# Abhipray/audio-codec

Measured on AMD Instinct MI355X. Metric: audio channel-frames/s encode (48 kHz, 1024-line long blocks, 128 kb/s/ch), higher is better.
Workload: dtype f64

## Files before the change

### audio-codec_amd/_lib.py

```python
import ctypes
import os

HERE = os.path.dirname(os.path.abspath(__file__))
LIB_PATH = os.environ.get("PACX_LIB") or os.path.join(HERE, "libpacx.so")

PACX_ABI_VERSION = 7
PCM_I16, PCM_F64 = 0, 1
FLAG_LAST, FLAG_CUR, FLAG_NEXT = 1, 2, 4
ST_SHORT, ST_ZERO_SUBBLOCK, ST_ALLOC_CAP, ST_VQ_UNDEFINED, ST_GUARD, ST_MALFORMED = 1, 2, 4, 8, 16, 32
ST_REF_RAISES = 64
ST_RATE_CAP = 128
RATE_STEP = 32
RATE_TARGET_GRID = 64
BAND_CAND = 16
PROFILE_MAX = 8193
SEG_CF_MAX = 1 << 40
E_ARG, E_UNSUPPORTED = -1, -2
REF_SCALAR_SBR_ERROR = "'numpy.int64' object does not support item assignment"
MAX_BANDS = 32
SUB = 8

c_double_p = ctypes.POINTER(ctypes.c_double)
c_int32_p = ctypes.POINTER(ctypes.c_int32)


class PacxSmrTables(ctypes.Structure):
    _fields_ = [
        ("hann", ctypes.c_void_p),
        ("tw_cos", ctypes.c_void_p),
        ("tw_sin", ctypes.c_void_p),
        ("fft_norm", ctypes.c_double),
        ("fft_freq_step", ctypes.c_double),
        ("bark", ctypes.c_void_p),
        ("quiet", ctypes.c_void_p),
        ("band_lower", ctypes.c_void_p),
        ("band_lines", ctypes.c_void_p),
        ("n_bands", ctypes.c_int32),
    ]


class PacxConfig(ctypes.Structure):
    _fields_ = [
        ("abi_version", ctypes.c_int32),
        ("device", ctypes.c_int32),
        ("sample_rate", ctypes.c_int32),
        ("n_lines_long", ctypes.c_int32),
        ("n_lines_short", ctypes.c_int32),
        ("n_scale_bits", ctypes.c_int32),
        ("n_mant_size_bits", ctypes.c_int32),
# ... 49 lines not shown
    "pacx_abi_version": (ctypes.c_int, []),
    "pacx_create": (ctypes.c_int, [ctypes.POINTER(PacxConfig), ctypes.POINTER(_P)]),
    "pacx_destroy": (None, [_P]),
    "pacx_last_error": (ctypes.c_char_p, [_P]),
    "pacx_band_stride": (ctypes.c_int, [_P]),
    "pacx_payload_stride": (ctypes.c_int, [_P]),
    "pacx_reserve": (ctypes.c_int, [_P, ctypes.c_int64]),
    "pacx_tables_exact": (ctypes.c_int, [_P]),
    "pacx_default_bands": (ctypes.c_int, [ctypes.c_int, ctypes.c_int, c_int32_p, c_int32_p]),
    "pacx_mdct_batch": (ctypes.c_int, [_P, ctypes.POINTER(PacxPcm), _P, ctypes.c_int, _P, _P, _P]),
    "pacx_smr_batch": (ctypes.c_int, [_P, ctypes.POINTER(PacxPcm), _P, ctypes.c_int, _P, _P, _P, _P]),
    "pacx_bitalloc_batch": (ctypes.c_int, [_P, ctypes.c_int64, ctypes.c_int, _P, ctypes.c_int, _P, _P, _P, _P]),
    "pacx_quantize_batch": (ctypes.c_int, [_P, ctypes.c_int64, _P, _P, _P, ctypes.c_int, _P, _P, _P]),
    "pacx_encode_batch": (ctypes.c_int, [_P, ctypes.POINTER(PacxPcm), _P, _P, _P, _P, _P, _P, _P]),
    "pacx_encode_pack_batch": (ctypes.c_int, [_P, ctypes.POINTER(PacxPcm), _P, _P, _P, _P, _P, _P, _P, _P, _P]),
    "pacx_encode_vq_batch": (ctypes.c_int, [_P, ctypes.POINTER(PacxPcm), _P, _P, _P, _P, _P, _P, _P, _P,
                                            ctypes.c_int32, _P]),
    "pacx_pack_batch": (ctypes.c_int, [_P, ctypes.c_int64, ctypes.c_int, _P, _P, _P, _P, _P, _P, _P, _P, _P]),
    "pacx_gather_body": (ctypes.c_int, [_P, ctypes.c_int64, _P, _P, _P, ctypes.c_int64, _P, _P]),
    "pacx_window_batch": (ctypes.c_int, [_P, ctypes.c_int, ctypes.c_int64, _P, _P, _P]),
    "pacx_window_table_batch": (ctypes.c_int, [_P, _P, ctypes.c_int, ctypes.c_int64, _P, _P, _P]),
    "pacx_quantize_uniform": (ctypes.c_int, [_P, ctypes.c_int64, _P, ctypes.c_int, _P, _P]),
    "pacx_scale_factor": (ctypes.c_int, [_P, ctypes.c_int64, _P, ctypes.c_int, ctypes.c_int, _P, _P]),
    "pacx_mantissa": (ctypes.c_int, [_P, ctypes.c_int64, _P, ctypes.c_int, ctypes.c_int, ctypes.c_int, _P, _P]),
    "pacx_dequantize_uniform": (ctypes.c_int, [_P, ctypes.c_int64, _P, ctypes.c_int, _P, _P]),
    "pacx_dequantize": (ctypes.c_int, [_P, ctypes.c_int64, _P, ctypes.c_int, ctypes.c_int, ctypes.c_int, _P, _P]),
    "pacx_mantissa_fp": (ctypes.c_int, [_P, ctypes.c_int64, _P, ctypes.c_int, ctypes.c_int, ctypes.c_int, _P, _P]),
    "pacx_dequantize_fp": (ctypes.c_int, [_P, ctypes.c_int64, _P, ctypes.c_int, ctypes.c_int, ctypes.c_int, _P, _P]),
    "pacx_imdct_batch": (ctypes.c_int, [_P, ctypes.c_int64, ctypes.c_int, _P, _P, _P]),
    "pacx_mdct_direct_batch": (ctypes.c_int, [_P, ctypes.c_int64, ctypes.c_int, ctypes.c_int, ctypes.c_int, _P, _P, _P]),
    "pacx_transient_detect_f64": (ctypes.c_int, [_P, ctypes.c_int64, ctypes.c_int, ctypes.c_int, _P, ctypes.c_double, _P, _P]),
    "pacx_unpack_batch": (ctypes.c_int, [_P, ctypes.c_int64, _P, ctypes.c_int, _P, _P, _P, _P, _P, _P, _P, _P, _P]),
    "pacx_set_side_fork": (ctypes.c_int, [_P, ctypes.c_int]),
    "pacx_smr_generic_batch": (ctypes.c_int, [_P, ctypes.c_int64, ctypes.c_int, _P, _P, ctypes.POINTER(PacxSmrTables), _P, _P,
                                              _P, _P]),
    "pacx_decode_batch": (ctypes.c_int, [_P, ctypes.c_int64, ctypes.c_int, _P, _P, _P, _P, _P, _P, _P, _P]),
    "pacx_decode_sbr_batch": (ctypes.c_int, [_P, ctypes.c_int64, ctypes.c_int, _P, _P, _P, _P, _P, ctypes.c_int, _P, _P,
                                             _P, _P, _P]),
    "pacx_decode_vq_batch": (ctypes.c_int, [_P, ctypes.c_int64, ctypes.c_int, _P, ctypes.c_int, _P, _P, _P, _P, _P,
                                            _P, _P, _P, _P, _P]),
    "pacx_transient_flags": (ctypes.c_int, [_P, ctypes.POINTER(PacxPcm), _P, _P, _P]),
    "pacx_bitalloc_generic": (ctypes.c_int, [_P, ctypes.c_int64, ctypes.c_int, _P, _P, ctypes.c_int, _P, _P, _P]),
    "pacx_index_body": (ctypes.c_int, [_P, _P, ctypes.c_int64, ctypes.c_int, ctypes.c_int, ctypes.c_int64, _P, _P, _P, _P]),
    "pacx_overlap_add_pcm": (ctypes.c_int, [_P, ctypes.c_int64, ctypes.c_int, _P, _P, ctypes.c_int, _P, _P]),
    "pacx_nmr_batch": (ctypes.c_int, [_P, ctypes.POINTER(PacxPcm), _P, _P, _P, _P, _P, _P, _P, _P]),
    "pacx_nmr_summary": (ctypes.c_int, [_P, ctypes.c_int64, ctypes.c_int, _P, _P, _P, _P]),
    "pacx_encode_pack_nmr_batch": (ctypes.c_int, [_P, ctypes.POINTER(PacxPcm), _P, ctypes.c_double, ctypes.c_double,
                                                  _P, _P, _P, _P, _P, _P, _P, _P, _P]),
    "pacx_encode_pack_budget_batch": (ctypes.c_int, [_P, ctypes.POINTER(PacxPcm), _P, _P, _P, _P, _P, _P, _P, _P, _P,
                                                     _P]),
    "pacx_rate_curve_layout": (ctypes.c_int, [_P, ctypes.c_double, c_int32_p, c_int32_p]),
    "pacx_rate_curve_batch": (ctypes.c_int, [_P, ctypes.POINTER(PacxPcm), _P, ctypes.c_double, ctypes.c_int32, _P, _P, _P,
                                             _P]),
    "pacx_rate_solve": (ctypes.c_int, [_P, ctypes.c_int64, ctypes.c_int32, ctypes.c_int32, _P, _P, _P, ctypes.c_int64,
                                       ctypes.c_double, ctypes.c_double, _P, _P, _P, _P, _P]),
    "pacx_band_curve_batch": (ctypes.c_int, [_P, ctypes.POINTER(PacxPcm), _P, ctypes.c_double, _P, _P, _P, _P]),
    "pacx_band_pick": (ctypes.c_int, [_P, ctypes.c_int64, _P, _P, _P, ctypes.c_double, _P, _P, _P, _P]),
    "pacx_band_solve": (ctypes.c_int, [_P, ctypes.c_int64, _P, _P, _P, ctypes.c_int64, ctypes.c_double, ctypes.c_double,
                                       _P, _P, _P, _P, _P]),
    "pacx_band_profile": (ctypes.c_int, [_P, ctypes.c_int64, _P, _P, _P, ctypes.c_double, ctypes.c_double, _P, _P]),
    "pacx_profile_solve": (ctypes.c_int, [_P, _P, ctypes.c_int64, ctypes.c_double, ctypes.c_double, _P, _P]),
    "pacx_band_profile_segments": (ctypes.c_int, [_P, ctypes.c_int64, _P, _P, _P, ctypes.c_int64, ctypes.c_int64,
                                                  ctypes.c_double, ctypes.c_double, _P, _P]),
    "pacx_profile_solve_segments": (ctypes.c_int, [_P, ctypes.c_int64, _P, _P, ctypes.c_double, ctypes.c_double, _P, _P,
                                                   _P]),
    "pacx_profile_clamp_add": (ctypes.c_int, [_P, ctypes.c_int64, _P, _P, ctypes.c_double, ctypes.c_double, _P, _P]),
# ... 75 lines not shown
```

### audio-codec_amd/csrc/k_misc.hip

```cpp
#include "pacx_launch.h"

__global__ void k_window(const double *__restrict__ win, long long n_rows, int len,
                         const double *__restrict__ x, double *__restrict__ y)
{
    const long long i = (long long)blockIdx.x * blockDim.x + threadIdx.x;
    if (i < n_rows * len)
        y[i] = win[i % len] * x[i];
}

__global__ void k_quant_elem(int op, long long n, const double *__restrict__ x, int scale, int a, int b,
                             int64_t *__restrict__ out)
{
    const long long i = (long long)blockIdx.x * blockDim.x + threadIdx.x;
    if (i >= n)
        return;
    const double v = x[i];
    if (op == 0) {
        const int64_t mag = pacx_quant_mag(fabs(v), a);
        out[i] = (v < 0.0 ? ((int64_t)1 << (a - 1)) : 0) + mag;
    } else if (op == 1) {
        out[i] = pacx_scale_factor(fabs(v), a, b);
    } else if (op == 2) {
        out[i] = pacx_mantissa(v, scale, a, b);
    } else {
// ... 299 lines not shown
    if (lane == 63) {
        ws[wv] = ss;
        wl[wv] = sl;
    }
    __syncthreads();
    int at_s = ss - ns, at_l = sl - nl, all_s = 0, all_l = 0;
#pragma unroll
    for (int w = 0; w < NW; ++w) {
        at_s += w < wv ? ws[w] : 0;
        at_l += w < wv ? wl[w] : 0;
        all_s += ws[w];
        all_l += wl[w];
    }
    for (int j = 0; j < per; ++j) {
        if (!((valid >> j) & 1ull))
            break;
        const long long f = f0 + j;
        if ((shorts >> j) & 1ull) {
            for (int c = 0; c < n_ch; ++c)
                list_short[at_s * n_ch + c] = (int32_t)(f * n_ch + c);
            ++at_s;
        } else {
            for (int c = 0; c < n_ch; ++c)
                list_long[at_l * n_ch + c] = (int32_t)(f * n_ch + c);
            ++at_l;
        }
    }
    if (tid == 0) {
        counts[0] = all_l * n_ch;
        counts[1] = all_s * n_ch;
    }
}

void pacx_k::pacx_launch_frame_lists(const uint8_t *flags, long long n_frames, int n_ch, int32_t *list_long,
                             int32_t *list_short, int32_t *counts, hipStream_t st)
{
    if (n_frames <= 0)
        return;
    if (n_frames <= LISTS_SMALL_MAX) {
        hipLaunchKernelGGL(k_frame_lists_small, dim3(1), dim3(LISTS_SMALL_THREADS), 0, st, flags, n_frames, n_ch, list_long,
                           list_short, counts);
        return;
    }
    (void)hipMemsetAsync(counts, 0, 2 * sizeof(int32_t), st);
    hipLaunchKernelGGL(k_frame_lists, dim3((unsigned)((n_frames + 255) / 256)), dim3(256), 0, st, flags, n_frames,
                       n_ch, list_long, list_short, counts);
}

void pacx_k::pacx_launch_transient_f64(long long n_blocks, int n_ch, int n, const double *blocks, double thresh, uint8_t *out,
                               hipStream_t st)
{
    if (n_blocks > 0)
        hipLaunchKernelGGL(k_transient_f64, dim3((unsigned)n_blocks), dim3(64), 0, st, n_blocks, n_ch, n, blocks, thresh,
                           out);
}

void pacx_k::pacx_launch_transient(const PacxPcmView &in, long long n_hops, int hop, uint8_t *transient,
                           uint8_t *flags, hipStream_t st)
{
    if (n_hops > 0)
        hipLaunchKernelGGL(k_transient, dim3((unsigned)n_hops), dim3(64), 0, st, in, n_hops, hop, transient);
    if (flags)
        hipLaunchKernelGGL(k_stream_flags, dim3((unsigned)((n_hops + 2 + 255) / 256)), dim3(256), 0, st,
                           transient, n_hops, flags);
}

// ... 40 lines not shown
```

### audio-codec_amd/csrc/k_quant.hip

```cpp
#include "pacx_launch.h"
#include "wave_fft.h"
#include "quant_dev.h"

__global__ __launch_bounds__(64) void k_bitalloc(PacxTables T, const uint8_t *__restrict__ flags, int n_ch,
                                                long long n_cf, int short_blocks, int mixed, int skip_long,
                                                const double *__restrict__ smr,
                                                int32_t *__restrict__ bit_alloc,
                                                uint32_t *__restrict__ status)
{
    __shared__ double cp[2][32];
    const int lane = threadIdx.x, half = lane >> 5, l = lane & 31;
    const bool dense = !short_blocks && !(mixed && flags);
    const long long unit = (long long)blockIdx.x * 2 + half;
    const long long cf = dense ? unit : unit / PACX_SUB;
    const int sb = dense ? 0 : (int)(unit % PACX_SUB);
    bool alive = cf < n_cf;
    const unsigned fl = (alive && flags) ? flags[cf / n_ch] : 0u;
    const bool is_short = mixed ? ((fl & 2u) != 0) : (short_blocks != 0);
    if (!is_short && (sb != 0 || skip_long == 1))
        alive = false;
    if (is_short && skip_long == 2)
        alive = false;
    const int nb = is_short ? T.nb_short : T.nb_long;
    const int32_t *__restrict__ n_lines = is_short ? T.band_lines_short
// ... 604 lines not shown
                                                     const long long *__restrict__ chunk_off,
                                                     long long *__restrict__ offs)
{
    __shared__ long long buf[256];
    const int t = threadIdx.x;
    const long long i = (long long)blockIdx.x * SCAN_CHUNK + t;
    const long long v = (i < n) ? rec_len(n_bytes[i]) : 0;
    buf[t] = v;
    __syncthreads();
    for (int off = 1; off < 256; off <<= 1) {
        const long long add = (t >= off) ? buf[t - off] : 0;
        __syncthreads();
        buf[t] += add;
        __syncthreads();
    }
    if (i < n)
        offs[i] = chunk_off[blockIdx.x] + buf[t] - v;
}

#define SCAN_SMALL_MAX 32768

__device__ __forceinline__ void copy_record(int nb, long long off, const uint8_t *__restrict__ src,
                                            uint8_t *__restrict__ body, long long capacity, int lane)
{
    if (nb <= 0 || off + nb + 4 > capacity)
        return;
    if (lane < 4)
        body[off + lane] = (uint8_t)((unsigned)nb >> (8 * lane));
    uint8_t *dst = body + off + 4;
    const int head = (int)((4 - ((uintptr_t)dst & 3)) & 3);
    if (lane < head && lane < nb)
        dst[lane] = src[lane];
    const int n_words = (nb - head) > 0 ? (nb - head) >> 2 : 0;
    for (int w = lane; w < n_words; w += 64) {
        const uint8_t *s = src + head + 4 * w;
        const unsigned v = (unsigned)s[0] | ((unsigned)s[1] << 8) | ((unsigned)s[2] << 16) | ((unsigned)s[3] << 24);
        *(unsigned *)(dst + head + 4 * w) = v;
    }
    const int done = head + 4 * n_words;
    if (done + lane < nb && lane < 4)
        dst[done + lane] = src[done + lane];
}

__global__ __launch_bounds__(64) void k_copy_body(const int32_t *__restrict__ n_bytes, long long n,
                                                 const long long *__restrict__ offs,
                                                 const uint8_t *__restrict__ payload, int payload_stride,
                                                 uint8_t *__restrict__ body, long long capacity)
{
    const long long i = blockIdx.x;
    if (i >= n)
        return;
    copy_record(n_bytes[i], offs[i], payload + i * (long long)payload_stride, body, capacity, threadIdx.x);
}

#define GATHER_REC 8
__global__ __launch_bounds__(256) void k_gather_small(const int32_t *__restrict__ n_bytes, long long n,
                                                     const uint8_t *__restrict__ payload, int payload_stride,
                                                     uint8_t *__restrict__ body, long long capacity,
                                                     long long *__restrict__ total)
{
    __shared__ int part[4];
    __shared__ int offs_s[GATHER_REC + 1];
    __shared__ int len_s[GATHER_REC];
    const int t = threadIdx.x, lane = t & 63, wv = t >> 6;
    const long long first = (long long)blockIdx.x * GATHER_REC;
    int acc = 0;
    const int4 *__restrict__ nb4 = (const int4 *)n_bytes;
    const int n4 = (int)(first >> 2);
#pragma unroll 8
    for (int j = t; j < n4; j += 256) {
        const int4 v = nb4[j];
        acc += (int)(rec_len(v.x) + rec_len(v.y) + rec_len(v.z) + rec_len(v.w));
    }
#pragma unroll
    for (int off = 32; off > 0; off >>= 1)
        acc += __shfl_xor(acc, off, 64);
    if (lane == 0)
        part[wv] = acc;
    __syncthreads();
    if (wv == 0) {
        const int base = part[0] + part[1] + part[2] + part[3];
        const int nb = (lane < GATHER_REC && first + lane < n) ? n_bytes[first + lane] : 0;
        const int len = (int)rec_len(nb);
        int incl = len;
#pragma unroll
        for (int off = 1; off < GATHER_REC; off <<= 1) {
            const int v = __shfl_up(incl, off, 64);
            if (lane >= off)
                incl += v;
        }
        if (lane < GATHER_REC) {
            offs_s[lane] = base + incl - len;
            len_s[lane] = nb;
        }
        if (lane == GATHER_REC - 1) {
            offs_s[GATHER_REC] = base + incl;
            if (total && first + GATHER_REC >= n)
                *total = (long long)(base + incl);
        }
    }
    __syncthreads();
    for (int r = wv; r < GATHER_REC && first + r < n; r += 4)
        copy_record(len_s[r], (long long)offs_s[r], payload + (first + r) * (long long)payload_stride, body,
                    capacity, lane);
}

void pacx_k::pacx_launch_bitalloc(const PacxTables &T, const uint8_t *flags, int n_ch, long long n_cf,
                          int short_blocks, int mixed, int skip_long, const double *smr, int32_t *bit_alloc,
                          uint32_t *status, hipStream_t st)
{
    if (n_cf <= 0)
        return;
    const bool dense = !short_blocks && !(mixed && flags);
    if (dense && skip_long == 1)
        return;
    const long long units = dense ? n_cf : n_cf * PACX_SUB;
    hipLaunchKernelGGL(k_bitalloc, dim3((unsigned)((units + 1) / 2)), dim3(64), 0, st, T, flags, n_ch,
                       n_cf, short_blocks, mixed, skip_long, smr, bit_alloc, status);
}

void pacx_k::pacx_launch_quantize(const PacxTables &T, const uint8_t *flags, int n_ch, long long n_cf,
                          int short_blocks, int mixed, const double *lines, const int32_t *overall,
                          int overall_stride, const int32_t *bit_alloc, int32_t *scale_factor,
                          int32_t *mantissa, hipStream_t st)
{
    if (n_cf <= 0)
        return;
    if (!short_blocks || mixed)
        hipLaunchKernelGGL((k_quantize<PACX_M_LONG>), dim3((unsigned)n_cf), dim3(64), 0, st, T, flags, n_ch,
                           n_cf, mixed, lines, overall, overall_stride, bit_alloc, scale_factor, mantissa);
    if (short_blocks || mixed)
        hipLaunchKernelGGL((k_quantize<PACX_M_SHORT>), dim3((unsigned)(n_cf * PACX_SUB)), dim3(64), 0, st, T,
                           flags, n_ch, n_cf * PACX_SUB, mixed, lines, overall, overall_stride, bit_alloc,
                           scale_factor, mantissa);
}

void pacx_k::pacx_launch_pack(const PacxTables &T, const uint8_t *flags, int n_ch, long long n_cf,
// ... 15 lines not shown
{
    if (n_cf <= 0)
        return;
    const int mixed = flags ? 1 : 0;
    if (skip_long != 1)
        hipLaunchKernelGGL(k_tail_long, dim3((unsigned)(mixed ? n_cf : (n_cf + 1) / 2)), dim3(64), 0, st, T, flags,
                           n_ch, n_cf, mixed, smr, lines, overall, bit_alloc, scale_factor, mantissa, status, payload,
                           payload_stride, n_bytes);
    if (skip_long == 2)
        return;
    if (mixed && list_short && T.nb_short <= 8) {
        hipLaunchKernelGGL(k_tail_short, dim3((unsigned)n_cf), dim3(256), 0, st, T, flags, n_ch, list_short,
                           count_short, smr, lines, overall, bit_alloc, scale_factor, mantissa, status, payload,
                           payload_stride, n_bytes);
    } else if (mixed) {
        const long long units = n_cf * PACX_SUB;
        hipLaunchKernelGGL(k_bitalloc, dim3((unsigned)((units + 1) / 2)), dim3(64), 0, st, T, flags, n_ch, n_cf,
                           0, 1, 1, smr, bit_alloc, status);
        hipLaunchKernelGGL((k_quantize<PACX_M_SHORT>), dim3((unsigned)units), dim3(64), 0, st, T, flags, n_ch,
                           units, 1, lines, overall, PACX_SUB, bit_alloc, scale_factor, mantissa);
        if (payload)
            hipLaunchKernelGGL(k_pack, dim3((unsigned)n_cf), dim3(64), 0, st, T, flags, n_ch, n_cf, overall,
                               scale_factor, bit_alloc, mantissa, status, payload, payload_stride, n_bytes, 1);
    }
}

void pacx_k::pacx_launch_gather(long long n_cf, const uint8_t *payload, int payload_stride,
                        const int32_t *n_bytes, long long *chunk_buf, long long *offs_buf, uint8_t *body,
                        long long capacity, long long *total, hipStream_t st)
{
    if (n_cf <= 0)
        return;
    if (n_cf <= SCAN_SMALL_MAX) {
        hipLaunchKernelGGL(k_gather_small, dim3((unsigned)((n_cf + GATHER_REC - 1) / GATHER_REC)), dim3(256), 0, st,
                           n_bytes, n_cf, payload, payload_stride, body, capacity, total);
        return;
    }
    const long long n_chunks = (n_cf + SCAN_CHUNK - 1) / SCAN_CHUNK;
    hipLaunchKernelGGL(k_scan_partial, dim3((unsigned)n_chunks), dim3(256), 0, st, n_bytes, n_cf, chunk_buf);
    hipLaunchKernelGGL(k_scan_chunks, dim3(1), dim3(64), 0, st, chunk_buf, n_chunks, total);
    hipLaunchKernelGGL(k_scan_offsets, dim3((unsigned)n_chunks), dim3(256), 0, st, n_bytes, n_cf, chunk_buf,
                       offs_buf);
    hipLaunchKernelGGL(k_copy_body, dim3((unsigned)n_cf), dim3(64), 0, st, n_bytes, n_cf, offs_buf, payload,
                       payload_stride, body, capacity);
}
```

### audio-codec_amd/csrc/pacx_api.hip

```cpp
#include <hip/hip_runtime.h>

#include <math.h>
#include <stdio.h>
#include <stdlib.h>
#include <string.h>

#include <cmath>
#include <string>
#include <vector>

#include "../../include/pacx.h"
#include "body_index.h"
#include "pacx_launch.h"
#include "pvq_dev.h"
#include "pacx_vq_tables.h"
#include "pacx_tables_gen.h"

using namespace pacx_k;

struct PacxOverrides {
    int split_short;
    int fuse_tail;
    int fuse_front;
    int vq_fuse_alloc;
    int vq_frame;
    int vq_bfs;
    int vq_dec_frame;
};

#define PACX_FUSE_FRONT_DEFAULT 1

static int env_override(const char *name, int lo, int hi)
{
    const char *e = getenv(name);
    if (!e || !*e)
        return -1;
    char *end;
    const long v = strtol(e, &end, 10);
    return (*end || v < lo || v > hi) ? -1 : (int)v;
}

static PacxOverrides read_overrides(void)
{
    PacxOverrides o;
    o.split_short = env_override("PACX_SPLIT_SHORT", 0, 0);
    o.fuse_tail = env_override("PACX_FUSE_TAIL", 0, 1);
    o.fuse_front = env_override("PACX_FUSE_FRONT", 0, 1);
    o.vq_fuse_alloc = env_override("PACX_VQ_FUSE_ALLOC", 0, 1);
    o.vq_frame = env_override("PACX_VQ_FRAME", 0, 0);
    o.vq_bfs = env_override("PACX_VQ_BFS", 0, 1 << 20);
    o.vq_dec_frame = env_override("PACX_VQ_DEC_FRAME", 0, 0);
    return o;
}

struct pacx_handle {
    int device;
    int n_cu;
    PacxOverrides force;
    PacxTables T;
    std::vector<void *> owned;
    long long ws_cf;
    double *ws_lines;
    double *ws_smr;
    PacxPeak *ws_peaks;
    int32_t *ws_npeaks;
    int32_t *ws_nkept;
    int32_t *ws_overall;
    long long *ws_chunks;
    long long *ws_offs;
    int32_t *ws_lists;
    long long ws_blocks_cf;
    double *ws_blocks;
    int fork_side;
    hipStream_t side_stream;
    hipEvent_t ev_fork, ev_join;
    hipStream_t short_stream;
    hipStream_t spare_stream;
    hipEvent_t ev_short_done, ev_lists;
    std::vector<char> vq_view;
    std::vector<char> vqdec_view;
    int tables_exact;
    long long ws_mant_cf;
    int32_t *ws_mant;
    long long ws_dec_cf;
    double *ws_dec_lines;
    uint8_t *ws_dec_sbr;
    uint32_t *ws_dec_status;
    double *ws_sbr_mean;
    long long ws_vq_cf;
    unsigned *ws_unit_words;
// ... 185 lines not shown
    if (cfg->device < 0 || cfg->device >= n_dev)
        return fail(nullptr, PACX_E_ARG, "pacx_create: device ordinal out of range");

    pacx_handle *h = new pacx_handle();
    h->device = cfg->device;
    h->force = read_overrides();
    h->tables_exact = 1;
    memset(&h->T, 0, sizeof(h->T));
    int rc = PACX_OK;
#define TRY(x) do { rc = (x); if (rc) { g_create_err = h->err; pacx_destroy(h); return rc; } } while (0)
    {
        hipError_t e = hipSetDevice(cfg->device);
        if (e != hipSuccess) {
            g_create_err = std::string("hipSetDevice: ") + hipGetErrorString(e);
            delete h;
            return PACX_E_HIP;
        }
    }
    if (hipStreamCreateWithFlags(&h->side_stream, hipStreamNonBlocking) != hipSuccess ||
        hipEventCreateWithFlags(&h->ev_fork, hipEventDisableTiming) != hipSuccess ||
        hipEventCreateWithFlags(&h->ev_join, hipEventDisableTiming) != hipSuccess ||
        hipStreamCreateWithFlags(&h->short_stream, hipStreamNonBlocking) != hipSuccess ||
        hipStreamCreateWithFlags(&h->spare_stream, hipStreamNonBlocking) != hipSuccess ||
        hipEventCreateWithFlags(&h->ev_short_done, hipEventDisableTiming) != hipSuccess ||
        hipEventCreateWithFlags(&h->ev_lists, hipEventDisableTiming) != hipSuccess) {
        g_create_err = "pacx_create: could not create the side stream / events";
        pacx_destroy(h);
        return PACX_E_HIP;
    }
    {
        hipDeviceProp_t prop;
        h->n_cu = (hipGetDeviceProperties(&prop, cfg->device) == hipSuccess && prop.multiProcessorCount > 0)
                      ? prop.multiProcessorCount : 256;
    }
    PacxTables &T = h->T;
    const int NL = PACX_N_LONG, NS = PACX_N_SHORT, ML = PACX_M_LONG, MS = PACX_M_SHORT;
    const double sr = cfg->sample_rate;

    std::vector<double> wl(4 * NL), ws(NS), hl(NL), hs(NS);
    if (cfg->win_long) {
        memcpy(wl.data(), cfg->win_long, sizeof(double) * 4 * NL);
    } else {
        const std::vector<double> sl = gen_table(PACX_GEN_SINE_LONG, NL), ss = gen_table(PACX_GEN_SINE_SHORT, NS);
        const int pad = NL / 4 - NS / 4;
        for (int i = 0; i < NL; ++i) {
            wl[i] = sl[i];
            double st;
            if (i < NL / 2) st = sl[i];
            else if (i < NL / 2 + pad) st = 1.0;
            else if (i < NL / 2 + pad + NS / 2) st = ss[NS / 2 + (i - NL / 2 - pad)];
            else st = 0.0;
            wl[NL + i] = st;
            double ssw;
            if (i < pad) ssw = 0.0;
            else if (i < pad + NS / 2) ssw = ss[i - pad];
            else if (i < pad + NS / 2 + 2 * pad) ssw = 1.0;
            else if (i < pad + NS + 2 * pad) ssw = ss[NS / 2 + (i - pad - NS / 2 - 2 * pad)];
            else ssw = 0.0;
            wl[3 * NL + i] = ssw;
        }
        for (int i = 0; i < NL; ++i)
            wl[2 * NL + i] = wl[NL + (NL - 1 - i)];
    }
    if (cfg->win_short) memcpy(ws.data(), cfg->win_short, sizeof(double) * NS);
    else ws = gen_table(PACX_GEN_SINE_SHORT, NS);
    if (cfg->hann_long) memcpy(hl.data(), cfg->hann_long, sizeof(double) * NL);
// ... 882 lines not shown
        return PACX_E_ARG;
    if (n_cf == 0)
        return PACX_OK;
    if (n_cf < 0 || n_channels < 1 || !overall_scale || !scale_factor || !bit_alloc || !mantissa || !payload ||
        !n_bytes)
        return fail(h, PACX_E_ARG, "pacx_pack_batch: bad argument");
    HIP_TRY(h, hipSetDevice(h->device));
    pacx_launch_pack(h->T, frame_flags, n_channels, n_cf, overall_scale, scale_factor, bit_alloc, mantissa,
                     status, payload, PACX_PAYLOAD_STRIDE, n_bytes, (hipStream_t)stream);
    return post_launch(h, "pacx_pack_batch");
}

extern "C" int pacx_gather_body(pacx_handle *h, int64_t n_cf, const uint8_t *payload, const int32_t *n_bytes,
                                uint8_t *body, int64_t body_capacity, int64_t *total_bytes, void *stream)
{
    if (!h)
        return PACX_E_ARG;
    if (n_cf == 0) {
        if (total_bytes)
            HIP_TRY(h, hipMemsetAsync(total_bytes, 0, sizeof(int64_t), (hipStream_t)stream));
        return PACX_OK;
    }
    if (n_cf < 0 || !payload || !n_bytes || !body || body_capacity < 0)
        return fail(h, PACX_E_ARG, "pacx_gather_body: bad argument");
    HIP_TRY(h, hipSetDevice(h->device));
    int rc = pacx_reserve(h, n_cf);
    if (rc)
        return rc;
    pacx_launch_gather(n_cf, payload, PACX_PAYLOAD_STRIDE, n_bytes, h->ws_chunks, h->ws_offs, body, body_capacity,
                       (long long *)total_bytes, (hipStream_t)stream);
    return post_launch(h, "pacx_gather_body");
}

extern "C" int pacx_window_batch(pacx_handle *h, int window, int64_t n_rows, const double *x, double *y,
                                 void *stream)
{
    if (!h)
        return PACX_E_ARG;
    if (n_rows < 0 || !x || !y)
        return fail(h, PACX_E_ARG, "pacx_window_batch: bad argument");
    const double *w;
    int len;
    switch (window) {
    case PACX_WIN_SINE: case PACX_WIN_START: case PACX_WIN_STOP: case PACX_WIN_STARTSTOP:
        w = h->T.win_long + window * PACX_N_LONG; len = PACX_N_LONG; break;
    case PACX_WIN_SINE_SHORT: w = h->T.win_short; len = PACX_N_SHORT; break;
    case PACX_WIN_HANN: w = h->T.hann_long; len = PACX_N_LONG; break;
    case PACX_WIN_HANN_SHORT: w = h->T.hann_short; len = PACX_N_SHORT; break;
    case PACX_WIN_KBD: w = h->T.kbd_long; len = PACX_N_LONG; break;
    case PACX_WIN_KBD_SHORT: w = h->T.kbd_short; len = PACX_N_SHORT; break;
    default: return fail(h, PACX_E_ARG, "pacx_window_batch: unknown window");
    }
    HIP_TRY(h, hipSetDevice(h->device));
    pacx_launch_window(w, n_rows, len, x, y, (hipStream_t)stream);
    return post_launch(h, "pacx_window_batch");
}

extern "C" int pacx_window_table_batch(pacx_handle *h, const double *table, int len, int64_t n_rows,
                                       const double *x, double *y, void *stream)
{
    if (!h)
        return PACX_E_ARG;
    if (n_rows < 0 || len < 1 || !table || !x || !y)
        return fail(h, PACX_E_ARG, "pacx_window_table_batch: bad argument");
    HIP_TRY(h, hipSetDevice(h->device));
    pacx_launch_window(table, n_rows, len, x, y, (hipStream_t)stream);
// ... 943 lines not shown
```

### audio-codec_amd/csrc/pacx_launch.h

```cpp
#ifndef PACX_LAUNCH_H
#define PACX_LAUNCH_H

#include "../../include/pacx.h"
#include "pacx_dev.h"

struct PvqTables;

namespace pacx_k {

void pacx_launch_mdct(const PacxTables &T, const PacxPcmView &in, int dtype, int fast,
                      const uint8_t *flags, long long n_cf, int short_blocks, int mixed, int prewin,
                      double *lines, int32_t *scale_out, int scale_stride, uint32_t *status,
                      hipStream_t st);
void pacx_launch_mdct_v2(const PacxTables &T, const PacxPcmView &in, const uint8_t *flags, long long n_cf,
                         int skip_cur, double *lines, int32_t *scale_out, int scale_stride,
                         uint32_t *status_init, int n_cu, const int32_t *cf_list, const int32_t *cf_count,
                         hipStream_t st);
void pacx_launch_mdct_x2(const PacxTables &T, const PacxPcmView &in, long long n_cf, double *lines,
                         int32_t *scale_out, int scale_stride, uint32_t *status_init, int n_cu, hipStream_t st);

void pacx_launch_side(const PacxTables &T, const PacxPcmView &in, int dtype, int fast,
                      const uint8_t *flags, long long n_cf, int short_blocks, int mixed,
                      PacxPeak *peaks, int32_t *n_peaks, int32_t *n_kept, double *sbr_mean,
                      int32_t *sbr_overall, hipStream_t st);
// ... 2 lines not shown
                            int32_t *n_kept, hipStream_t st);
void pacx_launch_mask(const PacxTables &T, const uint8_t *flags, int n_ch, long long n_cf,
                      int short_blocks, int mixed, const PacxPeak *peaks, const int32_t *n_peaks,
                      const double *lines, double *smr, double *thr_out, int n_cu,
                      const int32_t *list_long, const int32_t *list_short, const int32_t *counts,
                      const MaskTail *tail, hipStream_t st);
size_t pacx_smr_generic_lds(int n);
void pacx_launch_smr_generic(long long n_blocks, int n, int nb, const double *data, const double *lines,
                             const double *hann, const double *tw_cos, const double *tw_sin, double norm, double fstep,
                             const double *bark, const double *quiet, const int32_t *band_lower,
                             const int32_t *band_count, double *smr, double *thr_out, int32_t *n_peaks_out,
                             hipStream_t st);

void pacx_launch_bitalloc(const PacxTables &T, const uint8_t *flags, int n_ch, long long n_cf,
                          int short_blocks, int mixed, int skip_long, const double *smr, int32_t *bit_alloc,
                          uint32_t *status, hipStream_t st);
void pacx_launch_quantize(const PacxTables &T, const uint8_t *flags, int n_ch, long long n_cf,
                          int short_blocks, int mixed, const double *lines, const int32_t *overall,
                          int overall_stride, const int32_t *bit_alloc, int32_t *scale_factor,
                          int32_t *mantissa, hipStream_t st);
void pacx_launch_pack(const PacxTables &T, const uint8_t *flags, int n_ch, long long n_cf,
                      const int32_t *overall, const int32_t *scale_factor, const int32_t *bit_alloc,
                      const int32_t *mantissa, const uint32_t *status, uint8_t *payload,
                      int payload_stride, int32_t *n_bytes, hipStream_t st);
void pacx_launch_tail(const PacxTables &T, const uint8_t *flags, int n_ch, long long n_cf, const double *smr,
                      const double *lines, const int32_t *overall, int32_t *bit_alloc, int32_t *scale_factor,
                      int32_t *mantissa, uint32_t *status, uint8_t *payload, int payload_stride,
                      int32_t *n_bytes, const int32_t *list_short, const int32_t *count_short, int skip_long,
                      hipStream_t st);
void pacx_launch_gather(long long n_cf, const uint8_t *payload, int payload_stride,
                        const int32_t *n_bytes, long long *chunk_buf, long long *offs_buf, uint8_t *body,
                        long long capacity, long long *total, hipStream_t st);

void pacx_launch_frame_lists(const uint8_t *flags, long long n_frames, int n_ch, int32_t *list_long,
                             int32_t *list_short, int32_t *counts, hipStream_t st);
void pacx_launch_window(const double *win, long long n_rows, int len, const double *x, double *y,
                        hipStream_t st);
void pacx_launch_quant_elem(int op, long long n, const double *x, int scale, int a, int b, int64_t *out,
                            hipStream_t st);
void pacx_launch_dequant_elem(int op, long long n, const int64_t *codes, int scale, int a, int b, double *out,
                              hipStream_t st);
void pacx_launch_mdct_direct(long long n_rows, int a, int b, int inverse, const double *x, double *y, hipStream_t st);
void pacx_launch_bitalloc_generic(long long n, int nb, const int32_t *n_lines, const double *budget,
                                  int max_mant, const double *smr, int32_t *bits, hipStream_t st);
void pacx_launch_transient_f64(long long n_blocks, int n_ch, int n, const double *blocks, double thresh, uint8_t *out,
                               hipStream_t st);
void pacx_launch_transient(const PacxPcmView &in, long long n_hops, int hop, uint8_t *transient,
                           uint8_t *flags, hipStream_t st);

void pacx_launch_imdct_plain(const PacxTables &T, long long n_rows, int short_blocks, const double *lines,
                             double *blocks, hipStream_t st);
void pacx_launch_sbr_scalar_lines(const PacxTables &T, long long n_cf, const uint8_t *cf_flags,
                                  const int32_t *scale_factor, const int32_t *bit_alloc, const int32_t *mantissa,
                                  double *lines, uint8_t *sbr_flag, int routing, hipStream_t st);
void pacx_launch_unpack(const PacxTables &T, long long n_cf, const uint8_t *payload, int payload_stride,
                        const long long *offsets, const int32_t *n_bytes, uint8_t *flags_out, int32_t *overall,
                        int32_t *scale_factor, int32_t *bit_alloc, int32_t *mantissa, uint32_t *status,
                        hipStream_t st);
void pacx_launch_decode(const PacxTables &T, long long n_blocks, int n_ch, const uint8_t *cf_flags,
                        const int32_t *overall, const int32_t *scale_factor, const int32_t *bit_alloc,
                        const int32_t *mantissa, const double *lines_in, double *blocks, int16_t *pcm,
                        hipStream_t st);
void pacx_launch_ola_tail(long long n_blocks, int n_ch, const double *blocks, double *tail, int flush, int16_t *pcm,
                          hipStream_t st);

size_t pacx_index_ws_bytes(long long n_body, PacxIndexWs *ws);
// ... 152 lines not shown
```

### audio-codec_amd/engine.py

```python
import ctypes

import numpy as np
import torch

from . import _lib, tables
from .psychoac import ScaleFactorBands, AssignMDCTLinesFromFreqLimits

N_LONG, N_SHORT = 1024, 128


def _ptr(t):
    return ctypes.c_void_p(t.data_ptr()) if t is not None else None


class PcmView:

    def __init__(self, tensor, n_channels, n_frames, frame_stride, channel_stride,
                 sample_stride=1):
        if tensor.dtype == torch.int16:
            dt = _lib.PCM_I16
        elif tensor.dtype == torch.float64:
            dt = _lib.PCM_F64
        else:
            raise TypeError("PCM must be int16 codes or float64 signed fractions")
        if not tensor.is_cuda:
            raise ValueError("PCM tensor must live on the GPU")
        self.tensor = tensor
        self.n_channels, self.n_frames = int(n_channels), int(n_frames)
        if self.n_frames > 0 and self.n_channels > 0:
            last = (self.n_frames - 1) * max(int(frame_stride), 0) + (self.n_channels - 1) * max(int(channel_stride), 0) \
                + (2 * N_LONG - 1) * max(int(sample_stride), 0)
            have = tensor.untyped_storage().nbytes() // tensor.element_size() - tensor.storage_offset()
            if last >= have:
# ... 63 lines not shown
        cfg.win_short = f64("ws", tables.sine(2 * N_SHORT))
        cfg.hann_long = f64("hl", tables.hann(2 * N_LONG))
        cfg.hann_short = f64("hs", tables.hann(2 * N_SHORT))
        cfg.bark_long = f64("zl", tables.bark(tables.line_freqs(N_LONG, sr)))
        cfg.thresh_long = f64("tl", tables.thresh(tables.line_freqs(N_LONG, sr)))
        cfg.bark_short = f64("zs", tables.bark(tables.line_freqs(N_SHORT, sr)))
        cfg.thresh_short = f64("ts", tables.thresh(tables.line_freqs(N_SHORT, sr)))
        cfg.fft_norm_long = tables.fft_norm(2 * N_LONG)
        cfg.fft_norm_short = tables.fft_norm(2 * N_SHORT)
        cfg.fft_freq_step_long = tables.fft_freq_step(2 * N_LONG, sr)
        cfg.fft_freq_step_short = tables.fft_freq_step(2 * N_SHORT, sr)
        self.use_vq, self.use_sbr = bool(use_vq), bool(use_sbr)
        cfg.use_vq, cfg.use_sbr = int(self.use_vq), int(self.use_sbr)
        l_max = int(max(np.max(self.sfBands.nLines), np.max(self.sfBandsShort.nLines)))
        cfg.half_log2 = f64("hl2", tables.half_log2(l_max))
        cfg.vq_log2_tan = f64("lt", tables.vq_log2_tan())
        cfg.log_mu1 = tables.log_mu1()
        gw, gr = tables.sbr_gauss()
        cfg.sbr_gauss, cfg.sbr_gauss_radius = f64("gw", gw), gr
        cfg.line_freq_long = f64("lf", (np.arange(N_LONG) + 1 / 2) * (sr / (2 * N_LONG)))
        cfg.kbd_long = f64("kl", tables.kbd(2 * N_LONG))
        cfg.kbd_short = f64("ks", tables.kbd(2 * N_SHORT))
        cfg.guard = int(bool(guard))
        h = ctypes.c_void_p()
        rc = self.lib.pacx_create(ctypes.byref(cfg), ctypes.byref(h))
        _lib.check(self.lib, None, rc, "pacx_create")
        self.h = h
        self.band_stride = self.lib.pacx_band_stride(h)
        self.payload_stride = self.lib.pacx_payload_stride(h)

    def set_side_fork(self, enable):
        self._call("pacx_set_side_fork", int(bool(enable)))

    def close(self):
        if getattr(self, "h", None):
            self.lib.pacx_destroy(self.h)
            self.h = None

    def __del__(self):
        try:
            self.close()
        except Exception:
            pass

    def _stream(self):
        return ctypes.c_void_p(torch.cuda.current_stream(self.device).cuda_stream)

    def _empty(self, shape, dtype):
        return torch.empty(shape, dtype=dtype, device=self.device)

    def _call(self, name, *args):
        rc = getattr(self.lib, name)(self.h, *args)
        _lib.check(self.lib, self.h, rc, name)

    def reserve(self, n_cf):
        self._call("pacx_reserve", ctypes.c_int64(int(n_cf)))

    def flags_tensor(self, flags, n_frames):
        if flags is None:
            return None
        if isinstance(flags, torch.Tensor):
            t = flags.to(device=self.device, dtype=torch.uint8)
        else:
            a = np.asarray(flags)
            if a.ndim == 2:
                a = (a[:, 0] != 0) * 1 + (a[:, 1] != 0) * 2 + (a[:, 2] != 0) * 4
# ... 665 lines not shown
        return out

    def transient_detect(self, blocks, thresh=4.5):
        blocks = blocks.contiguous()
        n, n_ch, ln = blocks.shape
        out = self._empty((n,), torch.uint8)
        self._call("pacx_transient_detect_f64", ctypes.c_int64(n), int(n_ch), int(ln), _ptr(blocks),
                   ctypes.c_double(float(thresh)), _ptr(out), self._stream())
        return out

    def bit_alloc_generic(self, budget, max_mant_bits, n_lines, smr):
        smr = smr.contiguous()
        n, nb = smr.shape
        nl = torch.as_tensor(np.asarray(n_lines, dtype=np.int32), device=self.device)
        bits = self._empty((n, nb), torch.int32)
        self._call("pacx_bitalloc_generic", ctypes.c_int64(n), int(nb), _ptr(nl), _ptr(budget.contiguous()),
                   int(max_mant_bits), _ptr(smr), _ptr(bits), self._stream())
        return bits


class EncoderPool:

    def __init__(self, n, *args, **kwargs):
        self.encs = [Encoder(*args, **kwargs) for _ in range(max(1, int(n)))]
        dev = self.encs[0].device
        self.streams = [torch.cuda.Stream(device=dev) for _ in self.encs]
        self.done = [torch.cuda.Event() for _ in self.encs]
        self._turn = 0
        self._gate = self._gate_stream = None
        self._used = [False] * len(self.encs)
        if len(self.encs) > 1:
            for e in self.encs:
                e.set_side_fork(True)

    def __len__(self):
        return len(self.encs)

    def next(self):
        k = self._turn
        self._turn = (k + 1) % len(self.encs)
        return k

    def slot(self, k):
        pool = self

        class _Slot:
            def __enter__(self_inner):
                self_inner.ctx = torch.cuda.stream(pool.streams[k])
                self_inner.ctx.__enter__()
                return pool.encs[k]

            def __exit__(self_inner, *exc):
                pool.done[k].record(pool.streams[k])
                pool._used[k] = True
                return self_inner.ctx.__exit__(*exc)
        return _Slot()

    def align(self, delay_us=None):
        if len(self.encs) < 2:
            return
        if delay_us is None:
            delay_us = float(os.environ.get("PACX_POOL_GATE_US", "100"))
        if delay_us <= 0 or not hasattr(torch.cuda, "_sleep"):
            return
        dev = self.encs[0].device
        if self._gate is None:
            self._gate_stream = torch.cuda.Stream(device=dev)
            self._gate = torch.cuda.Event()
            t0, t1 = torch.cuda.Event(enable_timing=True), torch.cuda.Event(enable_timing=True)
            with torch.cuda.stream(self._gate_stream):
                torch.cuda._sleep(100_000)
                t0.record()
                torch.cuda._sleep(2_000_000)
                t1.record()
            t1.synchronize()
            self._cycles_per_us = 2_000_000 / max(t0.elapsed_time(t1) * 1e3, 1.0)
        with torch.cuda.stream(self._gate_stream):
            for k in range(len(self.encs)):
                if self._used[k]:
                    self._gate_stream.wait_event(self.done[k])
            torch.cuda._sleep(int(delay_us * self._cycles_per_us))
            self._gate.record(self._gate_stream)
        for s in self.streams:
            s.wait_event(self._gate)

    def wait(self, k, stream=None):
        (stream or torch.cuda.current_stream(self.encs[0].device)).wait_event(self.done[k])

    def synchronize(self):
        for s in self.streams:
            s.synchronize()

    def close(self):
        for e in self.encs:
            e.close()
```

### include/pacx.h

```cpp
#ifndef PACX_H
#define PACX_H

#include <stdint.h>

#ifdef __cplusplus
extern "C" {
#endif

#define PACX_ABI_VERSION 7

#define PACX_OK            0
#define PACX_E_ARG        -1
#define PACX_E_UNSUPPORTED -2
#define PACX_E_HIP        -3
#define PACX_E_NOMEM      -4

#define PACX_PCM_I16 0
#define PACX_PCM_F64 1

#define PACX_FLAG_LAST 1u
#define PACX_FLAG_CUR  2u
#define PACX_FLAG_NEXT 4u

#define PACX_WIN_SINE 0
// ... 139 lines not shown
                      void *stream);
int pacx_window_table_batch(pacx_handle *h, const double *table, int len, int64_t n_rows,
                            const double *x, double *y, void *stream);
int pacx_quantize_uniform(pacx_handle *h, int64_t n, const double *x, int n_bits, int64_t *codes,
                          void *stream);
int pacx_scale_factor(pacx_handle *h, int64_t n, const double *x, int n_scale_bits, int n_mant_bits,
                      int64_t *scale, void *stream);
int pacx_mantissa(pacx_handle *h, int64_t n, const double *x, int scale, int n_scale_bits,
                  int n_mant_bits, int64_t *mantissa, void *stream);
int pacx_dequantize_uniform(pacx_handle *h, int64_t n, const int64_t *codes, int n_bits, double *x,
                            void *stream);
int pacx_dequantize(pacx_handle *h, int64_t n, const int64_t *mantissa, int scale, int n_scale_bits,
                    int n_mant_bits, double *x, void *stream);
int pacx_mantissa_fp(pacx_handle *h, int64_t n, const double *x, int scale, int n_scale_bits,
                     int n_mant_bits, int64_t *mantissa, void *stream);
int pacx_dequantize_fp(pacx_handle *h, int64_t n, const int64_t *mantissa, int scale, int n_scale_bits,
                       int n_mant_bits, double *x, void *stream);
int pacx_imdct_batch(pacx_handle *h, int64_t n_rows, int mode, const double *lines, double *blocks,
                     void *stream);
int pacx_mdct_direct_batch(pacx_handle *h, int64_t n_rows, int a, int b, int inverse, const double *x,
                           double *y, void *stream);
int pacx_bitalloc_generic(pacx_handle *h, int64_t n, int n_bands, const int32_t *band_lines,
                          const double *budget, int max_mant_bits, const double *smr,
                          int32_t *bit_alloc, void *stream);

int pacx_transient_flags(pacx_handle *h, const pacx_pcm *hops, uint8_t *transient,
                         uint8_t *frame_flags, void *stream);

int pacx_transient_detect_f64(pacx_handle *h, int64_t n_blocks, int n_channels, int n_samples,
                              const double *blocks, double thresh, uint8_t *result, void *stream);

int pacx_set_side_fork(pacx_handle *h, int enable);

typedef struct pacx_smr_tables {
    const double *hann;
    const double *tw_cos, *tw_sin;
    double fft_norm;
    double fft_freq_step;
    const double *bark, *quiet;
    const int32_t *band_lower;
    const int32_t *band_lines;
    int32_t n_bands;
} pacx_smr_tables;
int pacx_smr_generic_batch(pacx_handle *h, int64_t n_blocks, int n_samples, const double *data,
                           const double *lines, const pacx_smr_tables *t, double *smr, double *threshold,
                           int32_t *n_peaks, void *stream);


int pacx_unpack_batch(pacx_handle *h, int64_t n_cf, const uint8_t *payload, int payload_stride,
                      const int64_t *offsets, const int32_t *n_bytes, uint8_t *cf_flags,
                      int32_t *overall_scale, int32_t *scale_factor, int32_t *bit_alloc,
                      int32_t *mantissa, uint32_t *status, void *stream);

int pacx_decode_batch(pacx_handle *h, int64_t n_blocks, int n_channels, const uint8_t *cf_flags,
                      const int32_t *overall_scale, const int32_t *scale_factor,
                      const int32_t *bit_alloc, const int32_t *mantissa, double *blocks,
                      int16_t *pcm, void *stream);

int pacx_decode_sbr_batch(pacx_handle *h, int64_t n_blocks, int n_channels, const uint8_t *cf_flags,
                          const int32_t *overall_scale, const int32_t *scale_factor,
                          const int32_t *bit_alloc, const int32_t *mantissa, int every_long_block,
                          double *lines, double *blocks, int16_t *pcm, uint32_t *status, void *stream);

int pacx_decode_vq_batch(pacx_handle *h, int64_t n_blocks, int n_channels, const uint8_t *payload,
                         int payload_stride, const int64_t *offsets, const int32_t *n_bytes,
                         uint8_t *cf_flags, int32_t *overall_scale, int32_t *bit_alloc, double *lines,
// ... 134 lines not shown
```

Measured before the change: 52.74 million.

## Add native stream-gate kernel and slim small-batch body gather to one wave

Replaces the torch _sleep-based pool gate, which needed a timing calibration, with a native HIP gate kernel that polls the wall clock for the requested delay. It also reworks k_gather_small into a single 64-lane wave handling 4 records, dropping shared memory and block barriers. The per-record byte copy is unrolled to four words per lane to add memory-level parallelism. Smaller blocks mean more blocks to launch, and the gate's delay now depends on the reported wall-clock rate.

New measurement: 54.07 million (median of 6 runs). 2.5% higher.

```diff
diff --git a/audio-codec_amd/_lib.py b/audio-codec_amd/_lib.py
--- a/audio-codec_amd/_lib.py
+++ b/audio-codec_amd/_lib.py
@@ -15,6 +15,7 @@
 BAND_CAND = 16
 PROFILE_MAX = 8193
 SEG_CF_MAX = 1 << 40
+GATE_MAX_US = 10000
 E_ARG, E_UNSUPPORTED = -1, -2
 REF_SCALAR_SBR_ERROR = "'numpy.int64' object does not support item assignment"
 MAX_BANDS = 32
@@ -130,6 +131,7 @@
     "pacx_transient_detect_f64": (ctypes.c_int, [_P, ctypes.c_int64, ctypes.c_int, ctypes.c_int, _P, ctypes.c_double, _P, _P]),
     "pacx_unpack_batch": (ctypes.c_int, [_P, ctypes.c_int64, _P, ctypes.c_int, _P, _P, _P, _P, _P, _P, _P, _P, _P]),
     "pacx_set_side_fork": (ctypes.c_int, [_P, ctypes.c_int]),
+    "pacx_stream_gate": (ctypes.c_int, [_P, ctypes.c_double, _P]),
     "pacx_smr_generic_batch": (ctypes.c_int, [_P, ctypes.c_int64, ctypes.c_int, _P, _P, ctypes.POINTER(PacxSmrTables), _P, _P,
                                               _P, _P]),
     "pacx_decode_batch": (ctypes.c_int, [_P, ctypes.c_int64, ctypes.c_int, _P, _P, _P, _P, _P, _P, _P, _P]),
diff --git a/audio-codec_amd/csrc/k_misc.hip b/audio-codec_amd/csrc/k_misc.hip
--- a/audio-codec_amd/csrc/k_misc.hip
+++ b/audio-codec_amd/csrc/k_misc.hip
@@ -355,6 +355,26 @@
     }
 }
 
+#define GATE_SLEEP 16
+__global__ __launch_bounds__(64) void k_stream_gate(unsigned long long ticks, unsigned long long max_polls)
+{
+    if (ticks == 0)
+        return;
+    const unsigned long long t0 = __builtin_amdgcn_s_memrealtime();
+    for (unsigned long long i = 0; i < max_polls; ++i) {
+        if (__builtin_amdgcn_s_memrealtime() - t0 >= ticks)
+            break;
+        __builtin_amdgcn_s_sleep(GATE_SLEEP);
+    }
+}
+
+void pacx_k::pacx_launch_stream_gate(double delay_us, double ticks_per_us, hipStream_t st)
+{
+    const unsigned long long ticks = (unsigned long long)ceil(delay_us * ticks_per_us);
+    const unsigned long long max_polls = (unsigned long long)ceil(delay_us * 20.0) + 64;
+    hipLaunchKernelGGL(k_stream_gate, dim3(1), dim3(64), 0, st, ticks, max_polls);
+}
+
 void pacx_k::pacx_launch_frame_lists(const uint8_t *flags, long long n_frames, int n_ch, int32_t *list_long,
                              int32_t *list_short, int32_t *counts, hipStream_t st)
 {
diff --git a/audio-codec_amd/csrc/k_quant.hip b/audio-codec_amd/csrc/k_quant.hip
--- a/audio-codec_amd/csrc/k_quant.hip
+++ b/audio-codec_amd/csrc/k_quant.hip
@@ -660,10 +660,22 @@
     if (lane < head && lane < nb)
         dst[lane] = src[lane];
     const int n_words = (nb - head) > 0 ? (nb - head) >> 2 : 0;
-    for (int w = lane; w < n_words; w += 64) {
-        const uint8_t *s = src + head + 4 * w;
-        const unsigned v = (unsigned)s[0] | ((unsigned)s[1] << 8) | ((unsigned)s[2] << 16) | ((unsigned)s[3] << 24);
-        *(unsigned *)(dst + head + 4 * w) = v;
+    for (int w0 = lane; w0 < n_words; w0 += 256) {
+        unsigned v[4] = {0u, 0u, 0u, 0u};
+#pragma unroll
+        for (int k = 0; k < 4; ++k) {
+            const int w = w0 + 64 * k;
+            if (w < n_words) {
+                const uint8_t *s = src + head + 4 * w;
+                v[k] = (unsigned)s[0] | ((unsigned)s[1] << 8) | ((unsigned)s[2] << 16) | ((unsigned)s[3] << 24);
+            }
+        }
+#pragma unroll
+        for (int k = 0; k < 4; ++k) {
+            const int w = w0 + 64 * k;
+            if (w < n_words)
+                *(unsigned *)(dst + head + 4 * w) = v[k];
+        }
     }
     const int done = head + 4 * n_words;
     if (done + lane < nb && lane < 4)
@@ -681,56 +693,48 @@
     copy_record(n_bytes[i], offs[i], payload + i * (long long)payload_stride, body, capacity, threadIdx.x);
 }
 
-#define GATHER_REC 8
-__global__ __launch_bounds__(256) void k_gather_small(const int32_t *__restrict__ n_bytes, long long n,
-                                                     const uint8_t *__restrict__ payload, int payload_stride,
-                                                     uint8_t *__restrict__ body, long long capacity,
-                                                     long long *__restrict__ total)
-{
-    __shared__ int part[4];
-    __shared__ int offs_s[GATHER_REC + 1];
-    __shared__ int len_s[GATHER_REC];
-    const int t = threadIdx.x, lane = t & 63, wv = t >> 6;
+#ifndef GATHER_REC
+#define GATHER_REC 4
+#endif
+static_assert(GATHER_REC >= 4 && GATHER_REC <= 64 && (GATHER_REC & (GATHER_REC - 1)) == 0,
+              "a wave's first record sits on a 16-byte boundary of n_bytes, one lane per record in the scan");
+__global__ __launch_bounds__(64) void k_gather_small(const int32_t *__restrict__ n_bytes, long long n,
+                                                    const uint8_t *__restrict__ payload, int payload_stride,
+                                                    uint8_t *__restrict__ body, long long capacity,
+                                                    long long *__restrict__ total)
+{
+    const int lane = threadIdx.x;
     const long long first = (long long)blockIdx.x * GATHER_REC;
+    const int nb = (lane < GATHER_REC && first + lane < n) ? n_bytes[first + lane] : 0;
     int acc = 0;
     const int4 *__restrict__ nb4 = (const int4 *)n_bytes;
     const int n4 = (int)(first >> 2);
 #pragma unroll 8
-    for (int j = t; j < n4; j += 256) {
+    for (int j = lane; j < n4; j += 64) {
         const int4 v = nb4[j];
         acc += (int)(rec_len(v.x) + rec_len(v.y) + rec_len(v.z) + rec_len(v.w));
     }
 #pragma unroll
     for (int off = 32; off > 0; off >>= 1)
         acc += __shfl_xor(acc, off, 64);
-    if (lane == 0)
-        part[wv] = acc;
-    __syncthreads();
-    if (wv == 0) {
-        const int base = part[0] + part[1] + part[2] + part[3];
-        const int nb = (lane < GATHER_REC && first + lane < n) ? n_bytes[first + lane] : 0;
-        const int len = (int)rec_len(nb);
-        int incl = len;
-#pragma unroll
-        for (int off = 1; off < GATHER_REC; off <<= 1) {
-            const int v = __shfl_up(incl, off, 64);
-            if (lane >= off)
-                incl += v;
-        }
-        if (lane < GATHER_REC) {
-            offs_s[lane] = base + incl - len;
-            len_s[lane] = nb;
-        }
-        if (lane == GATHER_REC - 1) {
-            offs_s[GATHER_REC] = base + incl;
-            if (total && first + GATHER_REC >= n)
-                *total = (long long)(base + incl);
-        }
-    }
-    __syncthreads();
-    for (int r = wv; r < GATHER_REC && first + r < n; r += 4)
-        copy_record(len_s[r], (long long)offs_s[r], payload + (first + r) * (long long)payload_stride, body,
-                    capacity, lane);
+    const int len = (int)rec_len(nb);
+    int incl = len;
+#pragma unroll
+    for (int off = 1; off < GATHER_REC; off <<= 1) {
+        const int v = __shfl_up(incl, off, 64);
+        if (lane >= off)
+            incl += v;
+    }
+    const int at = acc + incl - len;
+    if (total && lane == GATHER_REC - 1 && first + GATHER_REC >= n)
+        *total = (long long)(acc + incl);
+#pragma unroll
+    for (int r = 0; r < GATHER_REC; ++r) {
+        if (first + r >= n)
+            break;
+        copy_record(__shfl(nb, r, 64), (long long)__shfl(at, r, 64), payload + (first + r) * (long long)payload_stride,
+                    body, capacity, lane);
+    }
 }
 
 void pacx_k::pacx_launch_bitalloc(const PacxTables &T, const uint8_t *flags, int n_ch, long long n_cf,
@@ -812,7 +816,7 @@
     if (n_cf <= 0)
         return;
     if (n_cf <= SCAN_SMALL_MAX) {
-        hipLaunchKernelGGL(k_gather_small, dim3((unsigned)((n_cf + GATHER_REC - 1) / GATHER_REC)), dim3(256), 0, st,
+        hipLaunchKernelGGL(k_gather_small, dim3((unsigned)((n_cf + GATHER_REC - 1) / GATHER_REC)), dim3(64), 0, st,
                            n_bytes, n_cf, payload, payload_stride, body, capacity, total);
         return;
     }
diff --git a/audio-codec_amd/csrc/pacx_api.hip b/audio-codec_amd/csrc/pacx_api.hip
--- a/audio-codec_amd/csrc/pacx_api.hip
+++ b/audio-codec_amd/csrc/pacx_api.hip
@@ -56,6 +56,7 @@
 struct pacx_handle {
     int device;
     int n_cu;
+    double gate_ticks_per_us;
     PacxOverrides force;
     PacxTables T;
     std::vector<void *> owned;
@@ -307,6 +308,11 @@
         hipDeviceProp_t prop;
         h->n_cu = (hipGetDeviceProperties(&prop, cfg->device) == hipSuccess && prop.multiProcessorCount > 0)
                       ? prop.multiProcessorCount : 256;
+        int khz = 0;
+        if (hipDeviceGetAttribute(&khz, hipDeviceAttributeWallClockRate, cfg->device) != hipSuccess || khz <= 0)
+            khz = 100000;
+        h->gate_ticks_per_us = khz / 1000.0;
+        (void)hipGetLastError();
     }
     PacxTables &T = h->T;
     const int NL = PACX_N_LONG, NS = PACX_N_SHORT, ML = PACX_M_LONG, MS = PACX_M_SHORT;
@@ -1255,6 +1261,17 @@
     return post_launch(h, "pacx_gather_body");
 }
 
+extern "C" int pacx_stream_gate(pacx_handle *h, double delay_us, void *stream)
+{
+    if (!h)
+        return fail(nullptr, PACX_E_ARG, "pacx_stream_gate: null handle");
+    if (!(delay_us >= 0.0) || delay_us > PACX_GATE_MAX_US)
+        return fail(h, PACX_E_ARG, "pacx_stream_gate: delay_us must lie in [0, PACX_GATE_MAX_US]");
+    HIP_TRY(h, hipSetDevice(h->device));
+    pacx_launch_stream_gate(delay_us, h->gate_ticks_per_us, (hipStream_t)stream);
+    return post_launch(h, "pacx_stream_gate");
+}
+
 extern "C" int pacx_window_batch(pacx_handle *h, int window, int64_t n_rows, const double *x, double *y,
                                  void *stream)
 {
diff --git a/audio-codec_amd/csrc/pacx_launch.h b/audio-codec_amd/csrc/pacx_launch.h
--- a/audio-codec_amd/csrc/pacx_launch.h
+++ b/audio-codec_amd/csrc/pacx_launch.h
@@ -58,6 +58,7 @@
                         const int32_t *n_bytes, long long *chunk_buf, long long *offs_buf, uint8_t *body,
                         long long capacity, long long *total, hipStream_t st);
 
+void pacx_launch_stream_gate(double delay_us, double ticks_per_us, hipStream_t st);
 void pacx_launch_frame_lists(const uint8_t *flags, long long n_frames, int n_ch, int32_t *list_long,
                              int32_t *list_short, int32_t *counts, hipStream_t st);
 void pacx_launch_window(const double *win, long long n_rows, int len, const double *x, double *y,
diff --git a/audio-codec_amd/engine.py b/audio-codec_amd/engine.py
--- a/audio-codec_amd/engine.py
+++ b/audio-codec_amd/engine.py
@@ -1,4 +1,5 @@
 import ctypes
+import os
 
 import numpy as np
 import torch
@@ -128,6 +129,10 @@
     def set_side_fork(self, enable):
         self._call("pacx_set_side_fork", int(bool(enable)))
 
+    def stream_gate(self, delay_us, stream=None):
+        st = self._stream() if stream is None else ctypes.c_void_p(stream.cuda_stream)
+        self._call("pacx_stream_gate", ctypes.c_double(delay_us), st)
+
     def close(self):
         if getattr(self, "h", None):
             self.lib.pacx_destroy(self.h)
@@ -859,6 +864,7 @@
         if len(self.encs) > 1:
             for e in self.encs:
                 e.set_side_fork(True)
+            self.encs[0].stream_gate(0, self.streams[0])
 
     def __len__(self):
         return len(self.encs)
@@ -888,26 +894,16 @@
             return
         if delay_us is None:
             delay_us = float(os.environ.get("PACX_POOL_GATE_US", "100"))
-        if delay_us <= 0 or not hasattr(torch.cuda, "_sleep"):
+        if delay_us <= 0:
             return
-        dev = self.encs[0].device
         if self._gate is None:
-            self._gate_stream = torch.cuda.Stream(device=dev)
+            self._gate_stream = torch.cuda.Stream(device=self.encs[0].device)
             self._gate = torch.cuda.Event()
-            t0, t1 = torch.cuda.Event(enable_timing=True), torch.cuda.Event(enable_timing=True)
-            with torch.cuda.stream(self._gate_stream):
-                torch.cuda._sleep(100_000)
-                t0.record()
-                torch.cuda._sleep(2_000_000)
-                t1.record()
-            t1.synchronize()
-            self._cycles_per_us = 2_000_000 / max(t0.elapsed_time(t1) * 1e3, 1.0)
-        with torch.cuda.stream(self._gate_stream):
-            for k in range(len(self.encs)):
-                if self._used[k]:
-                    self._gate_stream.wait_event(self.done[k])
-            torch.cuda._sleep(int(delay_us * self._cycles_per_us))
-            self._gate.record(self._gate_stream)
+        for k in range(len(self.encs)):
+            if self._used[k]:
+                self._gate_stream.wait_event(self.done[k])
+        self.encs[0].stream_gate(delay_us, self._gate_stream)
+        self._gate.record(self._gate_stream)
         for s in self.streams:
             s.wait_event(self._gate)
 
diff --git a/include/pacx.h b/include/pacx.h
--- a/include/pacx.h
+++ b/include/pacx.h
@@ -195,6 +195,9 @@
 
 int pacx_set_side_fork(pacx_handle *h, int enable);
 
+#define PACX_GATE_MAX_US 10000
+int pacx_stream_gate(pacx_handle *h, double delay_us, void *stream);
+
 typedef struct pacx_smr_tables {
     const double *hann;
     const double *tw_cos, *tw_sin;
```
